# mariaalfaroc/omr_a2s_multimodal_transformer

Measured on AMD Instinct MI355X. Metric: training samples/sec, higher is better.
Workload: dtype bf16; 1 GPU; C2: image encoder (CNN) + 6-layer d_model=256 kern decoder, fwd+bwd+Adam, dropout on, teacher-forcing noise on; one sample = one score image + its token sequence; per_gpu_batch=32, global_batch=32, image=256x2048x1, seq_len=512, layers=6, d_model=256, vocab=6997, parallelism=dp1

## Files before the change

omr_a2s_multimodal_transformer_amd/csrc/gemm.hip:

```cpp
#include <type_traits>

#include "omr_common.h"
#include "omr_hip.h"

#include "gemm_steps.h"

namespace {

struct TileId { int m, n, split; bool valid; };
__device__ __forceinline__ TileId tile_of_block(const GemmArgs& g, int L) {
    const int slot = L >> 3;
    const long J = ((long)(slot / g.chunk) * 8 + (L & 7)) * g.chunk + slot % g.chunk;
    TileId t;
    t.valid = J < g.total;
    t.n = (int)(J % g.nt);
    t.m = (int)((J / g.nt) % g.mt);
    t.split = (int)(J / ((long)g.nt * g.mt));
    return t;
}

constexpr int BM = 128, BN = 128;

}

typedef unsigned char fp8;
typedef __attribute__((ext_vector_type(16))) unsigned char u8x16;
template <> struct Frag<fp8> {
    typedef u8x16 type;
    static constexpr int N = 16;
};
template <> __device__ __forceinline__ fp8 from_f32<fp8>(float x) { return (fp8)(__builtin_amdgcn_cvt_pk_fp8_f32(x, 0.f, 0, false) & 0xff); }
__device__ __forceinline__ float to_f32(fp8 x) { return __builtin_amdgcn_cvt_f32_fp8((int)x, 0); }
__device__ __forceinline__ void mma32(f32x16& acc, u8x16 a, u8x16 b) {
    long a2[2], b2[2];
    __builtin_memcpy(a2, &a, 16);
    __builtin_memcpy(b2, &b, 16);
    acc = __builtin_amdgcn_mfma_f32_32x32x16_fp8_fp8(a2[0], b2[0], acc, 0, 0, 0);
    acc = __builtin_amdgcn_mfma_f32_32x32x16_fp8_fp8(a2[1], b2[1], acc, 0, 0, 0);
}

namespace {

template <typename T> struct GemmCfg {
    static constexpr int VEC = Frag<T>::N;
    static constexpr int BK = 4 * KStep<T>::value;
    static constexpr int PITCH = BK + VEC;
    static constexpr int CHUNKS_PER_ROW = BK / VEC;
    static constexpr int NCH = BM * BK / VEC / 256;
    static constexpr int TPITCH = 128 + 32;
    static constexpr int OP_ELEMS = (BM * PITCH > BK * TPITCH) ? BM * PITCH : BK * TPITCH;
    static constexpr int CPITCH = 64 + 8;
    static constexpr int LDS_ELEMS = (2 * OP_ELEMS > 4 * 64 * CPITCH) ? 2 * OP_ELEMS : 4 * 64 * CPITCH;
};
template <typename T, bool TR> struct UseTrRead { static constexpr bool value = TR && std::is_same<T, bf16>::value; };

template <typename T> __device__ __forceinline__ typename Frag<T>::type load_chunk_guard(
    const T* p, int valid)
{
    typedef typename Frag<T>::type F;
    if (valid <= 0) return frag_zero<T>();
    F v = *reinterpret_cast<const F*>(p);
    if (valid < Frag<T>::N) {
#pragma unroll
        for (int i = 0; i < Frag<T>::N; ++i)
            if (i >= valid) v[i] = from_f32<T>(0.f);
    }
    return v;
}

template <typename T, bool TR> struct Stager {
    typedef GemmCfg<T> Cfg;
    typedef typename Frag<T>::type F;
    F r[Cfg::NCH];
    __device__ __forceinline__ void load(const T* src, long ld, int row0, int nrows, int k0, int kend, int tid) {
#pragma unroll
        for (int i = 0; i < Cfg::NCH; ++i) {
            const int c = tid + i * 256;
            if (!TR) {
                const int row = c / Cfg::CHUNKS_PER_ROW, kc = (c % Cfg::CHUNKS_PER_ROW) * Cfg::VEC;
                const int gr = row0 + row, gk = k0 + kc;
                r[i] = (gr < nrows) ? load_chunk_guard<T>(src + (long)gr * ld + gk, kend - gk) : frag_zero<T>();
            } else {
                constexpr int CPR = 128 / Cfg::VEC;
                const int k = c / CPR, rc = (c % CPR) * Cfg::VEC;
                const int gk = k0 + k, gr = row0 + rc;
                r[i] = (gk < kend) ? load_chunk_guard<T>(src + (long)gk * ld + gr, nrows - gr) : frag_zero<T>();
            }
        }
    }
    __device__ __forceinline__ void store(T* lds, int tid) {
#pragma unroll
        for (int i = 0; i < Cfg::NCH; ++i) {
            const int c = tid + i * 256;
            if (!TR) {
                const int row = c / Cfg::CHUNKS_PER_ROW, kc = (c % Cfg::CHUNKS_PER_ROW) * Cfg::VEC;
                *reinterpret_cast<F*>(lds + row * Cfg::PITCH + kc) = r[i];
            } else {
                constexpr int CPR = 128 / Cfg::VEC;
                const int k = c / CPR, rc = (c % CPR) * Cfg::VEC;
                if constexpr (UseTrRead<T, TR>::value) {
                    *reinterpret_cast<F*>(lds + k * Cfg::TPITCH + rc) = r[i];
                } else {
#pragma unroll
                    for (int e = 0; e < Cfg::VEC; ++e) lds[(rc + e) * Cfg::PITCH + k] = r[i][e];
                }
            }
        }
    }
    __device__ __forceinline__ void add_colsum(float (&cs)[Cfg::VEC]) {
#pragma unroll
        for (int i = 0; i < Cfg::NCH; ++i)
#pragma unroll
            for (int e = 0; e < Cfg::VEC; ++e) cs[e] += to_f32(r[i][e]);
    }
};

template <typename T, bool TR>
__device__ __forceinline__ typename Frag<T>::type load_frag(const T* lds, int row0, int ks, int lane) {
    typedef GemmCfg<T> Cfg;
    typedef typename Frag<T>::type F;
    if constexpr (UseTrRead<T, TR>::value) {
        const int q = (lane & 15) >> 2, col = row0 + ((lane >> 4) & 1) * 16 + (lane & 3) * 4, k = ks + 8 * (lane >> 5) + q;
        return tr_frag_bf16(lds + k * Cfg::TPITCH + col, 4 * Cfg::TPITCH * (int)sizeof(T));
    } else {
        return *reinterpret_cast<const F*>(&lds[(row0 + (lane & 31)) * Cfg::PITCH + ks + (lane >> 5) * Cfg::VEC]);
    }
}

template <typename T, typename TC, bool TA, bool TB, bool FULLK>
__device__ __forceinline__ void gemm_body(const GemmArgs& g, const int block_index) {
    typedef GemmCfg<T> Cfg;
    typedef typename Frag<T>::type F;
    constexpr bool SWAP = std::is_same<TC, bf16>::value && std::is_same<T, bf16>::value;
    __shared__ __attribute__((aligned(16))) T smem[Cfg::LDS_ELEMS];
    T* As = smem;
    T* Bs = smem + Cfg::OP_ELEMS;

    const int tid = threadIdx.x, lane = tid & 63, wave = tid >> 6;
    const int wm = wave >> 1, wn = wave & 1;
    const TileId tile = tile_of_block(g, block_index);
    if (!tile.valid) return;
    const int m0 = tile.m * BM, n0 = tile.n * BN;
    const int kbeg = tile.split * g.ksplit_len;
    const int kend = min(g.K, kbeg + g.ksplit_len);
    const T* A = (const T*)g.A;
    const T* B = (const T*)g.B + grp_delta(g, 1, n0) * g.ldb;

    __shared__ __attribute__((aligned(16))) float sbias[BN];
    if constexpr (SWAP) {
        if (tid < BN) {
            const float* bp = g.bias ? g.bias + grp_delta(g, 1, n0) : nullptr;
            sbias[tid] = (bp != nullptr && tile.split == 0 && n0 + tid < g.N) ? bp[n0 + tid] : 0.f;
        }
    }

    f32x16 acc[2][2];
    acc_clear(acc);
    float cs[Cfg::VEC];
#pragma unroll
    for (int e = 0; e < Cfg::VEC; ++e) cs[e] = 0.f;
    const bool do_cs = TA && g.colsum_a != nullptr && tile.n == 0;
    auto mma_slab = [&]() {
#pragma unroll
        for (int ks = 0; ks < Cfg::BK; ks += KStep<T>::value) {
            F a[2], b[2];
#pragma unroll
            for (int i = 0; i < 2; ++i) a[i] = load_frag<T, TA>(As, wm * 64 + i * 32, ks, lane);
#pragma unroll
            for (int j = 0; j < 2; ++j) b[j] = load_frag<T, TB>(Bs, wn * 64 + j * 32, ks, lane);
#pragma unroll
            for (int i = 0; i < 2; ++i)
#pragma unroll
                for (int j = 0; j < 2; ++j) {
                    if constexpr (SWAP) mma32(acc[i][j], b[j], a[i]);
                    else mma32(acc[i][j], a[i], b[j]);
                }
        }
    };
    if constexpr (FULLK) {
        Stager<T, TA> fa[4];
        Stager<T, TB> fb[4];
        const int nk = (kend - kbeg + Cfg::BK - 1) / Cfg::BK;
#pragma unroll
        for (int sl = 0; sl < 4; ++sl)
            if (sl < nk) {
                fa[sl].load(A, g.lda, m0, g.M, kbeg + sl * Cfg::BK, kend, tid);
                fb[sl].load(B + grp_delta(g, 2, kbeg + sl * Cfg::BK) * g.ldb, g.ldb, n0, g.N, kbeg + sl * Cfg::BK, kend, tid);
            }
#pragma unroll
        for (int sl = 0; sl < 4; ++sl)
            if (sl < nk) {
                if (sl) __syncthreads();
                fa[sl].store(As, tid);
                fb[sl].store(Bs, tid);
                __syncthreads();
                mma_slab();
            }
        __syncthreads();
    } else {
        Stager<T, TA> sa;
        Stager<T, TB> sb;
        sa.load(A, g.lda, m0, g.M, kbeg, kend, tid);
        sb.load(B + grp_delta(g, 2, kbeg) * g.ldb, g.ldb, n0, g.N, kbeg, kend, tid);
        if (do_cs) sa.add_colsum(cs);
        sa.store(As, tid);
        sb.store(Bs, tid);
        __syncthreads();

        for (int k0 = kbeg; k0 < kend; k0 += Cfg::BK) {
            const bool more = (k0 + Cfg::BK) < kend;
            if (more) {
                sa.load(A, g.lda, m0, g.M, k0 + Cfg::BK, kend, tid);
                sb.load(B + grp_delta(g, 2, k0 + Cfg::BK) * g.ldb, g.ldb, n0, g.N, k0 + Cfg::BK, kend, tid);
            }
            mma_slab();
            __syncthreads();
            if (more) {
                if (do_cs) sa.add_colsum(cs);
                sa.store(As, tid);
                sb.store(Bs, tid);
                __syncthreads();
            }
        }
    }

    if (do_cs) {
        constexpr int CPR = 128 / Cfg::VEC;
        float* red = reinterpret_cast<float*>(smem);
        if (tid < 128) red[tid] = 0.f;
        __syncthreads();
        const int ml = (tid % CPR) * Cfg::VEC;
#pragma unroll
        for (int e = 0; e < Cfg::VEC; ++e) atomicAdd(&red[ml + e], cs[e]);
        __syncthreads();
        if (tid < 128 && m0 + tid < g.M) atomicAdd(&g.colsum_a[m0 + tid + grp_delta(g, 3, m0)], red[tid]);
        __syncthreads();
    }

    TC* C = (TC*)g.C + grp_delta(g, 3, m0) * g.ldc;
    const float* biasp = g.bias ? g.bias + grp_delta(g, 1, n0) : nullptr;
    if constexpr (SWAP) {
        T* Cs = smem + wave * (64 * Cfg::CPITCH);
        const int hsel = 4 * (lane >> 5);
#pragma unroll
        for (int j = 0; j < 2; ++j) {
            float bv[16];
#pragma unroll
            for (int q = 0; q < 4; ++q) {
                const f32x4 b4 = *reinterpret_cast<const f32x4*>(&sbias[wn * 64 + j * 32 + 8 * q + hsel]);
                bv[4 * q] = b4[0]; bv[4 * q + 1] = b4[1]; bv[4 * q + 2] = b4[2]; bv[4 * q + 3] = b4[3];
            }
#pragma unroll
            for (int i = 0; i < 2; ++i) {
                T* crow = Cs + (i * 32 + (lane & 31)) * Cfg::CPITCH + j * 32 + hsel;
#pragma unroll
                for (int q = 0; q < 4; ++q)
                    *reinterpret_cast<bf16x4*>(crow + 8 * q) = pack_ct4(acc[i][j], q, [&](float v, int e) {
                        v = v + bv[4 * q + e];
                        if (g.relu) v = fmaxf(v, 0.f);
                        return v;
                    });
            }
        }
        const bool vec_ok = (g.ldc % 8) == 0 && (((uintptr_t)C) & 15) == 0;
#pragma unroll
        for (int it = 0; it < 8; ++it) {
            const int c = lane + it * 64, row = c >> 3, kc = (c & 7) * 8;
            const int gr = m0 + wm * 64 + row, gc = n0 + wn * 64 + kc;
            if (gr >= g.M || gc >= g.N) continue;
            bf16x8 v = *reinterpret_cast<const bf16x8*>(Cs + row * Cfg::CPITCH + kc);
            if (g.drop_thresh) {
#pragma unroll
                for (int e = 0; e < 8; ++e)
                    v[e] = drop_keep(g.drop_seed, (uint64_t)((long)gr * g.ldc + gc + e), g.drop_thresh) ? (bf16)((float)v[e] * g.drop_scale) : (bf16)0.f;
            }
            TC* dst = C + (long)gr * g.ldc + gc;
            if (vec_ok && gc + 8 <= g.N && !g.accum) {
                *reinterpret_cast<bf16x8*>(dst) = v;
            } else {
#pragma unroll
                for (int e = 0; e < 8; ++e)
                    if (gc + e < g.N) dst[e] = g.accum ? (bf16)((float)dst[e] + (float)v[e]) : v[e];
            }
        }
    } else {
        const int col_l = lane & 31;
#pragma unroll
        for (int j = 0; j < 2; ++j) {
            const int col = n0 + wn * 64 + j * 32 + col_l;
            if (col >= g.N) continue;
            const float bv = (biasp != nullptr && tile.split == 0) ? biasp[col] : 0.f;
#pragma unroll
            for (int i = 0; i < 2; ++i) {
#pragma unroll
                for (int r = 0; r < 16; ++r) {
                    const int row = m0 + wm * 64 + i * 32 + acc_row(r, lane);
                    if (row >= g.M) continue;
                    float v = acc[i][j][r];
                    if constexpr (std::is_same<T, fp8>::value) v *= g.scale_a[row] * g.scale_b[col];
                    v += bv;
                    if (g.relu) v = fmaxf(v, 0.f);
                    if constexpr (!TA) {
                        if (g.drop_thresh) v = drop_keep(g.drop_seed, (uint64_t)((long)row * g.ldc + col), g.drop_thresh) ? to_f32(from_f32<TC>(v)) * g.drop_scale : 0.f;
                    }
                    TC* dst = C + (long)row * g.ldc + col;
                    if (g.atomic) {
                        if constexpr (sizeof(TC) == 4) atomicAdd((float*)dst, v);
                    } else if (g.accum) {
                        *dst = from_f32<TC>(to_f32(*dst) + v);
                    } else {
                        *dst = from_f32<TC>(v);
                    }
                }
            }
        }
    }
}

template <typename T, typename TC, bool TA, bool TB, bool FULLK>
__global__ __launch_bounds__(256) void gemm_kernel(GemmArgs g) {
    gemm_body<T, TC, TA, TB, FULLK>(g, blockIdx.x);
}

struct GemmPlan { int ksplit_len, splits, mt, nt, total, chunk, blocks; };
template <typename D, typename S> __host__ __device__ __forceinline__ void put_plan(D& d, const S& s) {
    d.ksplit_len = s.ksplit_len; d.mt = s.mt; d.nt = s.nt; d.chunk = s.chunk; d.total = s.total;
}

struct DwProb {
    const void* A; const void* B; float* C; float* colsum;
    int M, N, K, ksplit_len; int lda, ldb, ldc, block0; int nt, mt, chunk, total; int grp, grp_stride, grp_base, pad;
};
constexpr int DW_MAX = 24;
struct DwGroup { int nprob, pad; DwProb p[DW_MAX]; };
static_assert(sizeof(DwGroup) == 2312, "the table travels as kernel arguments: DwProb stays the compact record, not a GemmArgs (160 bytes each)");

template <typename T>
__global__ __launch_bounds__(256) void gemm_dw_grouped_kernel(DwGroup grp) {
    int pi = 0;
    for (int i = 1; i < grp.nprob; ++i) pi = ((int)blockIdx.x >= grp.p[i].block0) ? i : pi;
    const DwProb& q = grp.p[pi];
    GemmArgs g;
    g.A = q.A; g.B = q.B; g.C = q.C; g.M = q.M; g.N = q.N; g.K = q.K; g.lda = q.lda; g.ldb = q.ldb; g.ldc = q.ldc;
    g.accum = 1; g.atomic = 1; g.colsum_a = q.colsum;
    put_plan(g, q);
    g.grp = q.grp; g.grp_stride = q.grp_stride; g.grp_base = q.grp_base; g.grp_operand = q.grp ? 3 : 0;
    gemm_body<T, float, true, true, false>(g, (int)blockIdx.x - q.block0);
}

GemmPlan gemm_plan(int M, int N, int K, int bk, int want_splits) {
    GemmPlan p;
    p.ksplit_len = cdiv(cdiv(K, want_splits), bk) * bk;
    p.splits = cdiv(K, p.ksplit_len);
    p.mt = cdiv(M, BM); p.nt = cdiv(N, BN);
    p.total = p.nt * p.mt * p.splits;
    p.chunk = p.splits > 1 ? p.nt * p.mt : p.nt;
    p.blocks = cdiv(p.total / p.chunk, 8) * 8 * p.chunk;
    return p;
}

template <typename T, typename TC> int launch(GemmArgs g, int ta, int tb, const GemmPlan& p, hipStream_t s) {
    put_plan(g, p);
    constexpr bool CAN_FULLK = !std::is_same<T, fp8>::value;
    const bool fullk = CAN_FULLK && !ta && p.splits == 1 && g.K <= 4 * GemmCfg<T>::BK;
    void (*kernel)(GemmArgs) = nullptr;
    if constexpr (!CAN_FULLK) kernel = (ta || tb) ? nullptr : gemm_kernel<T, TC, false, false, false>;
    else if (ta) kernel = tb ? gemm_kernel<T, TC, true, true, false> : gemm_kernel<T, TC, true, false, false>;
    else if (tb) kernel = fullk ? gemm_kernel<T, TC, false, true, true> : gemm_kernel<T, TC, false, true, false>;
    else kernel = fullk ? gemm_kernel<T, TC, false, false, true> : gemm_kernel<T, TC, false, false, false>;
    if (!kernel) return OMR_ERR_UNSUPPORTED;
    hipLaunchKernelGGL(kernel, dim3((unsigned)p.blocks), dim3(256), 0, s, g);
    OMR_CHECK_LAUNCH();
    return OMR_OK;
}

}

extern "C" int omr_gemm(int dtype, int c_dtype, int transA, int transB, int M, int N, int K, const void* A, long lda,
                        const void* B, long ldb, void* C, long ldc, const float* bias, int relu, int accumulate,
                        int split_k, float* colsum_a, float drop_p, unsigned long long drop_seed, int row_group, int row_group_stride,
                        int row_group_base, int row_group_operand, void* stream) {
    if (M <= 0 || N <= 0 || K <= 0 || !A || !B || !C) return OMR_ERR_ARG;
    const int vec = dtype == OMR_BF16 ? 8 : 4;
    if (lda % vec || ldb % vec) return OMR_ERR_ARG;
    if (((uintptr_t)A & 15) || ((uintptr_t)B & 15)) return OMR_ERR_ARG;
    if (split_k < 1) split_k = 1;
    if (split_k > 1 && c_dtype != OMR_F32) return OMR_ERR_ARG;
    GemmArgs g;
    g.A = A; g.B = B; g.C = C; g.bias = bias; g.M = M; g.N = N; g.K = K; g.lda = lda; g.ldb = ldb; g.ldc = ldc;
    g.relu = relu; g.accum = accumulate; g.atomic = split_k > 1; g.colsum_a = colsum_a;
    if (drop_p < 0.f || drop_p >= 1.f || (drop_p > 0.f && (split_k > 1 || accumulate || transA))) return OMR_ERR_ARG;
    if (row_group_operand) {
        if (row_group_operand < 1 || row_group_operand > 3 || row_group <= 0 || row_group % 128 || row_group_stride < row_group || row_group_base < 0) return OMR_ERR_ARG;
        if ((row_group_operand == 2 && !transB) || (row_group_operand == 1 && transB)) return OMR_ERR_ARG;
        g.grp = row_group; g.grp_stride = row_group_stride; g.grp_base = row_group_base; g.grp_operand = row_group_operand;
    }
    g.drop_thresh = OMR_DROP_THRESH16(drop_p); g.drop_scale = 1.f / (1.f - drop_p); g.drop_seed = drop_seed;
    if (colsum_a && !transA) return OMR_ERR_ARG;
    const GemmPlan plan = gemm_plan(M, N, K, dtype == OMR_BF16 ? 64 : 32, split_k);
    hipStream_t s = (hipStream_t)stream;
    const GemmCall call = {dtype, c_dtype, transA, transB, plan.splits, drop_p};
    int rc = omr_gemm_panel_bf16(call, g, s);
    if (rc == OMR_ERR_UNSUPPORTED) rc = omr_gemm_tall_bf16(call, g, s);
    if (rc != OMR_ERR_UNSUPPORTED) return rc;
    if (dtype == OMR_BF16) {
        if (c_dtype == OMR_BF16) return launch<bf16, bf16>(g, transA, transB, plan, s);
        return launch<bf16, float>(g, transA, transB, plan, s);
    } else if (dtype == OMR_F32) {
        if (c_dtype != OMR_F32) return OMR_ERR_UNSUPPORTED;
        return launch<float, float>(g, transA, transB, plan, s);
    }
    return OMR_ERR_UNSUPPORTED;
}

extern "C" int omr_linear_wgrad_grouped(int dtype, int nprob, const omr_dw_problem* probs, void* stream) {
    if (nprob <= 0 || !probs) return OMR_ERR_ARG;
    if (dtype != OMR_BF16 && dtype != OMR_F32) return OMR_ERR_UNSUPPORTED;
    const int vec = dtype == OMR_BF16 ? 8 : 4, bk = dtype == OMR_BF16 ? 64 : 32;
    long tiles_total = 0;
    for (int i = 0; i < nprob; ++i) tiles_total += (long)cdiv(probs[i].n_out, BM) * cdiv(probs[i].n_in, BN);
    hipStream_t s = (hipStream_t)stream;
    for (int base = 0; base < nprob; base += DW_MAX) {
        DwGroup grp;
        grp.nprob = nprob - base < DW_MAX ? nprob - base : DW_MAX; grp.pad = 0;
        int block0 = 0;
        for (int i = 0; i < grp.nprob; ++i) {
            const omr_dw_problem& q = probs[base + i];
            if (!q.dy || !q.x || !q.dw || q.rows <= 0 || q.n_out <= 0 || q.n_in <= 0) return OMR_ERR_ARG;
            if (q.ld_dy % vec || q.ld_x % vec || ((uintptr_t)q.dy & 15) || ((uintptr_t)q.x & 15)) return OMR_ERR_ARG;
            if (q.row_group && (q.row_group % 128 || q.row_group_stride < q.row_group || q.row_group_base < 0)) return OMR_ERR_ARG;
            DwProb& d = grp.p[i];
            d.A = q.dy; d.B = q.x; d.C = q.dw; d.colsum = q.db;
            d.M = q.n_out; d.N = q.n_in; d.K = q.rows; d.lda = (int)q.ld_dy; d.ldb = (int)q.ld_x; d.ldc = (int)q.ld_dw;
            long want = (2048L + tiles_total - 1) / tiles_total;
            long maxs = (q.rows + 511) / 512;
            if (want > maxs) want = maxs;
            if (want < 1) want = 1;
            const GemmPlan plan = gemm_plan(d.M, d.N, d.K, bk, (int)want);
            put_plan(d, plan);
            d.block0 = block0;
            block0 += plan.blocks;
            d.grp = q.row_group; d.grp_stride = q.row_group_stride; d.grp_base = q.row_group_base; d.pad = 0;
        }
        if (dtype == OMR_BF16) hipLaunchKernelGGL((gemm_dw_grouped_kernel<bf16>), dim3((unsigned)block0), dim3(256), 0, s, grp);
        else hipLaunchKernelGGL((gemm_dw_grouped_kernel<float>), dim3((unsigned)block0), dim3(256), 0, s, grp);
        OMR_CHECK_LAUNCH();
    }
    return OMR_OK;
}

namespace {
template <typename T>
__global__ __launch_bounds__(256) void quantize_rows_fp8_kernel(const T* __restrict__ x, long ldx, fp8* __restrict__ q, long ldq, float* __restrict__ scale,
                                                                int M, int K) {
    const int lane = threadIdx.x & 63;
    const long row = blockIdx.x * (long)(blockDim.x >> 6) + (threadIdx.x >> 6);
    if (row >= M) return;
    const T* xr = x + row * ldx;
    float mx = 0.f;
    for (int k = lane; k < K; k += 64) mx = fmaxf(mx, fabsf(to_f32(xr[k])));
    mx = wave_max(mx);
    const float sc = mx > 0.f ? mx / 448.f : 1.f;
    for (int k = lane; k < K; k += 64) q[row * ldq + k] = from_f32<fp8>(to_f32(xr[k]) / sc);
    if (lane == 0) scale[row] = sc;
}
}

extern "C" int omr_quantize_rows_fp8(int dtype, const void* x, long ldx, unsigned char* q, long ldq, float* scale, int M, int K, void* stream) {
    if (M <= 0 || K <= 0 || !x || !q || !scale || ldx < K || ldq < K) return OMR_ERR_ARG;
    hipStream_t s = (hipStream_t)stream;
    if (dtype == OMR_BF16) hipLaunchKernelGGL((quantize_rows_fp8_kernel<bf16>), cdiv(M, 4), 256, 0, s, (const bf16*)x, ldx, q, ldq, scale, M, K);
    else if (dtype == OMR_F32) hipLaunchKernelGGL((quantize_rows_fp8_kernel<float>), cdiv(M, 4), 256, 0, s, (const float*)x, ldx, q, ldq, scale, M, K);
    else return OMR_ERR_UNSUPPORTED;
    OMR_CHECK_LAUNCH();
    return OMR_OK;
}

extern "C" int omr_gemm_fp8(int c_dtype, int M, int N, int K, const unsigned char* A8, long lda, const float* scale_a, const unsigned char* W8, long ldb,
                            const float* scale_w, void* C, long ldc, const float* bias, int relu, void* stream) {
    if (M <= 0 || N <= 0 || K <= 0 || !A8 || !W8 || !C || !scale_a || !scale_w) return OMR_ERR_ARG;
    if (lda % 16 || ldb % 16 || ((uintptr_t)A8 & 15) || ((uintptr_t)W8 & 15)) return OMR_ERR_ARG;
    GemmArgs g;
    g.A = A8; g.B = W8; g.C = C; g.bias = bias; g.M = M; g.N = N; g.K = K; g.lda = lda; g.ldb = ldb; g.ldc = ldc;
    g.relu = relu; g.scale_a = scale_a; g.scale_b = scale_w;
    const GemmPlan plan = gemm_plan(M, N, K, GemmCfg<fp8>::BK, 1);
    hipStream_t s = (hipStream_t)stream;
    if (c_dtype == OMR_BF16) return launch<fp8, bf16>(g, 0, 0, plan, s);
    if (c_dtype == OMR_F32) return launch<fp8, float>(g, 0, 0, plan, s);
    return OMR_ERR_UNSUPPORTED;
}
```

omr_a2s_multimodal_transformer_amd/csrc/gemm_args.h:

```cpp
#pragma once
#include <hip/hip_runtime.h>

struct GemmArgs {
    const void* A = nullptr; const void* B = nullptr; void* C = nullptr; const float* bias = nullptr;
    int M = 0, N = 0, K = 0; long lda = 0, ldb = 0, ldc = 0;
    int relu = 0, accum = 0, atomic = 0, ksplit_len = 0;
    float* colsum_a = nullptr;
    int mt = 0, nt = 0, chunk = 0, total = 0;
    unsigned drop_thresh = 0; float drop_scale = 1.f; unsigned long long drop_seed = 0;
    int grp = 0, grp_stride = 0, grp_base = 0, grp_operand = 0;
    const float* scale_a = nullptr; const float* scale_b = nullptr;
};
static_assert(sizeof(GemmArgs) == 160, "GemmArgs travels as kernel arguments");

struct GemmCall { int dtype, c_dtype, trans_a, trans_b, splits; float drop_p; };
int omr_gemm_panel_bf16(const GemmCall& call, const GemmArgs& g, hipStream_t s);
int omr_gemm_tall_bf16(const GemmCall& call, const GemmArgs& g, hipStream_t s);
```

Before: 1391 samples/s.

## Add stream-K grouped weight-gradient kernel for n_in=256 bf16 problems

Routes bf16 weight-gradient problems with n_in equal to 256 to a new persistent kernel. It splits the flattened (problem, output tile, k-tile) item space evenly across at most one workgroup per CU. Each 1024-thread workgroup double-buffers 64-row slabs of dy and x in 128 KB of LDS via async DMA, accumulates a 256x256 tile with MFMA, and flushes partial results and the bias column-sum with atomics at tile boundaries. The aim is better load balance and fewer small launches than the 128x128 split-K grouped kernel for the decoder's d_model=256 linears. In exchange it relies on fp32 atomics, which make the summation order nondeterministic, and on high LDS use per workgroup.

```diff
diff --git a/omr_a2s_multimodal_transformer_amd/csrc/gemm.hip b/omr_a2s_multimodal_transformer_amd/csrc/gemm.hip
--- a/omr_a2s_multimodal_transformer_amd/csrc/gemm.hip
+++ b/omr_a2s_multimodal_transformer_amd/csrc/gemm.hip
@@ -1,4 +1,5 @@
 #include <type_traits>
+#include <vector>
 
 #include "omr_common.h"
 #include "omr_hip.h"
@@ -417,18 +418,25 @@
     if (nprob <= 0 || !probs) return OMR_ERR_ARG;
     if (dtype != OMR_BF16 && dtype != OMR_F32) return OMR_ERR_UNSUPPORTED;
     const int vec = dtype == OMR_BF16 ? 8 : 4, bk = dtype == OMR_BF16 ? 64 : 32;
+    for (int i = 0; i < nprob; ++i) {
+        const omr_dw_problem& q = probs[i];
+        if (!q.dy || !q.x || !q.dw || q.rows <= 0 || q.n_out <= 0 || q.n_in <= 0) return OMR_ERR_ARG;
+        if (q.ld_dy % vec || q.ld_x % vec || ((uintptr_t)q.dy & 15) || ((uintptr_t)q.x & 15)) return OMR_ERR_ARG;
+        if (q.row_group && (q.row_group % 128 || q.row_group_stride < q.row_group || q.row_group_base < 0)) return OMR_ERR_ARG;
+    }
+    hipStream_t s = (hipStream_t)stream;
+    std::vector<omr_dw_problem> rest((size_t)nprob);
+    const int rc = omr_dw_stream_bf16(dtype, nprob, probs, rest.data(), &nprob, s);
+    if (rc != OMR_OK) return rc;
+    probs = rest.data();
     long tiles_total = 0;
     for (int i = 0; i < nprob; ++i) tiles_total += (long)cdiv(probs[i].n_out, BM) * cdiv(probs[i].n_in, BN);
-    hipStream_t s = (hipStream_t)stream;
     for (int base = 0; base < nprob; base += DW_MAX) {
         DwGroup grp;
         grp.nprob = nprob - base < DW_MAX ? nprob - base : DW_MAX; grp.pad = 0;
         int block0 = 0;
         for (int i = 0; i < grp.nprob; ++i) {
             const omr_dw_problem& q = probs[base + i];
-            if (!q.dy || !q.x || !q.dw || q.rows <= 0 || q.n_out <= 0 || q.n_in <= 0) return OMR_ERR_ARG;
-            if (q.ld_dy % vec || q.ld_x % vec || ((uintptr_t)q.dy & 15) || ((uintptr_t)q.x & 15)) return OMR_ERR_ARG;
-            if (q.row_group && (q.row_group % 128 || q.row_group_stride < q.row_group || q.row_group_base < 0)) return OMR_ERR_ARG;
             DwProb& d = grp.p[i];
             d.A = q.dy; d.B = q.x; d.C = q.dw; d.colsum = q.db;
             d.M = q.n_out; d.N = q.n_in; d.K = q.rows; d.lda = (int)q.ld_dy; d.ldb = (int)q.ld_x; d.ldc = (int)q.ld_dw;
diff --git a/omr_a2s_multimodal_transformer_amd/csrc/gemm_args.h b/omr_a2s_multimodal_transformer_amd/csrc/gemm_args.h
--- a/omr_a2s_multimodal_transformer_amd/csrc/gemm_args.h
+++ b/omr_a2s_multimodal_transformer_amd/csrc/gemm_args.h
@@ -16,3 +16,6 @@
 struct GemmCall { int dtype, c_dtype, trans_a, trans_b, splits; float drop_p; };
 int omr_gemm_panel_bf16(const GemmCall& call, const GemmArgs& g, hipStream_t s);
 int omr_gemm_tall_bf16(const GemmCall& call, const GemmArgs& g, hipStream_t s);
+
+struct omr_dw_problem;
+int omr_dw_stream_bf16(int dtype, int nprob, const omr_dw_problem* probs, omr_dw_problem* rest, int* nrest, hipStream_t s);
diff --git a/omr_a2s_multimodal_transformer_amd/csrc/gemm_dw_stream.hip b/omr_a2s_multimodal_transformer_amd/csrc/gemm_dw_stream.hip
--- /dev/null
+++ b/omr_a2s_multimodal_transformer_amd/csrc/gemm_dw_stream.hip
@@ -0,0 +1,198 @@
+#include <climits>
+#include "omr_common.h"
+#include "omr_hip.h"
+#include "gemm_steps.h"
+#include "dma_common.h"
+#include "launch_setup.h"
+
+namespace {
+
+constexpr int TM = 256, NIN = 256;
+constexpr int BK = 64, KS = BK / 16;
+constexpr int ROWB = NIN * 2;
+constexpr int SLAB = BK * ROWB, STAGE = 2 * SLAB, SMEM = 2 * STAGE;
+constexpr int COPIES = BK / 2 / 16;
+constexpr int ITEMS_PER_WG = 8;
+static_assert(SMEM == 131072 && COPIES == 2, "two 64 KB stages, 2 + 2 copies per wave and k-tile");
+
+struct DwsProb {
+    const bf16* dy; const bf16* x; float* dw; float* db;
+    int rows, n_out, ld_dy, ld_x, ld_dw, grp, grp_stride, grp_base, item0, pad;
+};
+constexpr int DWS_MAX = 40;
+struct DwsTable { int nprob, nitems; DwsProb p[DWS_MAX]; };
+static_assert(sizeof(DwsProb) == 72 && sizeof(DwsTable) == 2888, "the table travels as kernel arguments (4 KB at the most)");
+
+struct Cursor { int p, t, kt, nk, tiles; };
+__device__ __forceinline__ void cursor_problem(Cursor& c, const DwsTable& tab, int p) {
+    c.p = p; c.nk = (tab.p[p].rows + BK - 1) / BK; c.tiles = (tab.p[p].n_out + TM - 1) / TM;
+}
+__device__ __forceinline__ void cursor_next(Cursor& c, const DwsTable& tab) {
+    if (++c.kt < c.nk) return;
+    c.kt = 0;
+    if (++c.t < c.tiles) return;
+    c.t = 0;
+    cursor_problem(c, tab, c.p + 1);
+}
+
+__device__ __forceinline__ float sum8(bf16x8 f) {
+    const uint4 u = __builtin_bit_cast(uint4, f);
+    const unsigned w[4] = {u.x, u.y, u.z, u.w};
+    float s = 0.f;
+#pragma unroll
+    for (int e = 0; e < 4; ++e) s += __uint_as_float(w[e] << 16) + __uint_as_float(w[e] & 0xffff0000u);
+    return s;
+}
+
+__global__ __launch_bounds__(1024) void gemm_dw_grouped_stream_kernel(DwsTable tab) {
+    extern __shared__ __attribute__((aligned(16))) unsigned char smem[];
+    const int tid = threadIdx.x, lane = tid & 63, hh = lane >> 5, wave = __builtin_amdgcn_readfirstlane(tid >> 6), wm = wave >> 2, wn = wave & 3;
+    const unsigned lds0 = lds_address(smem);
+    const int G = (int)gridDim.x;
+    const int it0 = (int)((long)blockIdx.x * tab.nitems / G), it1 = (int)((long)(blockIdx.x + 1) * tab.nitems / G);
+    if (it0 >= it1) return;
+
+    const int q = (lane & 15) >> 2, pc = ((lane >> 4) & 1) * 16 + (lane & 3) * 4;
+    int d_off[2], x_off[2];
+#pragma unroll
+    for (int i = 0; i < 2; ++i) {
+        const int cd = wm * 64 + i * 32 + pc, cx = wn * 64 + i * 32 + pc;
+        d_off[i] = (8 * hh + q) * ROWB + (((cd >> 3) ^ (q << 2)) << 4) + (cd & 7) * 2;
+        x_off[i] = SLAB + (8 * hh + q) * ROWB + (((cx >> 3) ^ (q << 2)) << 4) + (cx & 7) * 2;
+    }
+    int kr[COPIES], cb[COPIES];
+#pragma unroll
+    for (int u = 0; u < COPIES; ++u) {
+        kr[u] = (COPIES * wave + u) * 2 + (lane >> 5);
+        cb[u] = (lane & 31) ^ ((kr[u] & 3) << 2);
+    }
+    auto issue = [&](const Cursor& c, int stage) {
+        const DwsProb& pr = tab.p[c.p];
+        const unsigned st = lds0 + stage * STAGE;
+        const int k0 = c.kt * BK, last_row = pr.rows - 1, last_chunk = ((pr.n_out + 7) >> 3) - 1, c0 = c.t * (TM / 8);
+#pragma unroll
+        for (int u = 0; u < COPIES; ++u) {
+            const long row = min(k0 + kr[u], last_row);
+            dma16(pr.dy + row * pr.ld_dy + min(c0 + cb[u], last_chunk) * 8, st + (COPIES * wave + u) * 1024);
+            dma16(pr.x + row * pr.ld_x + cb[u] * 8, st + SLAB + (COPIES * wave + u) * 1024);
+        }
+    };
+
+    Cursor cc;
+    {
+        int p = 0;
+        for (int i = 1; i < tab.nprob; ++i) p = (it0 >= tab.p[i].item0) ? i : p;
+        cursor_problem(cc, tab, p);
+        const int local = it0 - tab.p[p].item0;
+        cc.t = local / cc.nk; cc.kt = local % cc.nk;
+    }
+    Cursor ci = cc;
+
+    f32x16 acc[2][2];
+    acc_clear(acc);
+    const bool db_wave = wn == wm;
+    float dbs[2] = {0.f, 0.f};
+
+    issue(ci, 0);
+    for (int it = it0; it < it1; ++it) {
+        const int stage = (it - it0) & 1;
+        dma_wait_barrier<0>();
+        if (it + 1 < it1) { cursor_next(ci, tab); issue(ci, stage ^ 1); }
+        unsigned char* st = smem + stage * STAGE;
+        const int valid = tab.p[cc.p].rows - cc.kt * BK;
+        if (valid < BK) {
+#pragma unroll
+            for (int e = 0; e < 2 * SLAB / 16 / 1024; ++e) {
+                const int ch = tid + e * 1024;
+                if (((ch >> 5) & (BK - 1)) >= valid) *reinterpret_cast<uint4*>(st + ch * 16) = make_uint4(0, 0, 0, 0);
+            }
+            lds_barrier();
+        }
+#pragma unroll
+        for (int ks = 0; ks < KS; ++ks) {
+            bf16x8 df[2], xf[2];
+#pragma unroll
+            for (int i = 0; i < 2; ++i) df[i] = tr_frag_bf16(st + d_off[i] + ks * 16 * ROWB, 4 * ROWB);
+#pragma unroll
+            for (int j = 0; j < 2; ++j) xf[j] = tr_frag_bf16(st + x_off[j] + ks * 16 * ROWB, 4 * ROWB);
+#pragma unroll
+            for (int i = 0; i < 2; ++i)
+#pragma unroll
+                for (int j = 0; j < 2; ++j) mma32(acc[i][j], df[i], xf[j]);
+            if (db_wave) {
+#pragma unroll
+                for (int i = 0; i < 2; ++i) dbs[i] += sum8(df[i]);
+            }
+        }
+        const bool last = it + 1 == it1;
+        if (cc.kt + 1 == cc.nk || last) {
+            const DwsProb& pr = tab.p[cc.p];
+            const int m0 = cc.t * TM;
+            const long delta = pr.grp ? (long)(m0 / pr.grp) * (pr.grp_stride - pr.grp) + pr.grp_base : 0;
+            float* dwt = pr.dw + (m0 + delta) * (long)pr.ld_dw + wn * 64 + (lane & 31);
+            const int n_left = pr.n_out - m0;
+#pragma unroll
+            for (int i = 0; i < 2; ++i)
+#pragma unroll
+                for (int r = 0; r < 16; ++r) {
+                    const int ml = wm * 64 + i * 32 + (r >> 2) * 8 + hh * 4 + (r & 3);
+                    if (ml < n_left) {
+#pragma unroll
+                        for (int j = 0; j < 2; ++j) atomicAdd(dwt + (long)ml * pr.ld_dw + j * 32, acc[i][j][r]);
+                    }
+                }
+            acc_clear(acc);
+            if (db_wave) {
+#pragma unroll
+                for (int i = 0; i < 2; ++i) {
+                    const float v = dbs[i] + __shfl_xor(dbs[i], 32);
+                    const int ml = wm * 64 + i * 32 + (lane & 31);
+                    if (pr.db && hh == 0 && ml < n_left) atomicAdd(pr.db + m0 + delta + ml, v);
+                    dbs[i] = 0.f;
+                }
+            }
+        }
+        if (!last) cursor_next(cc, tab);
+    }
+}
+
+bool accepts(int dtype, const omr_dw_problem& q) {
+    if (dtype != OMR_BF16 || q.n_in != NIN || q.rows <= 0 || q.n_out <= 0) return false;
+    if (q.ld_dy % 8 || q.ld_x % 8 || ((uintptr_t)q.dy & 15) || ((uintptr_t)q.x & 15)) return false;
+    if (q.ld_dy < q.n_out || q.ld_x < NIN || q.ld_dw < NIN || q.ld_dy > INT_MAX || q.ld_x > INT_MAX || q.ld_dw > INT_MAX) return false;
+    if (q.row_group && q.row_group % TM) return false;
+    return (long)cdiv(q.n_out, TM) * cdiv(q.rows, BK) < (1L << 24);
+}
+
+}
+
+int omr_dw_stream_bf16(int dtype, int nprob, const omr_dw_problem* probs, omr_dw_problem* rest, int* nrest, hipStream_t s) {
+    *nrest = 0;
+    DwsTable tab;
+    tab.nprob = 0; tab.nitems = 0;
+    auto launch = [&]() -> int {
+        if (!tab.nprob) return OMR_OK;
+        static std::atomic<int> ready{0};
+        if (!omr_launch_setup(ready, (const void*)gemm_dw_grouped_stream_kernel, SMEM, true)) return OMR_ERR_LAUNCH;
+        const int want = tab.nitems / ITEMS_PER_WG, grid = want < 1 ? 1 : want > OMR_NUM_CU ? OMR_NUM_CU : want;
+        hipLaunchKernelGGL(gemm_dw_grouped_stream_kernel, dim3(grid), dim3(1024), SMEM, s, tab);
+        OMR_CHECK_LAUNCH();
+        tab.nprob = 0; tab.nitems = 0;
+        return OMR_OK;
+    };
+    for (int i = 0; i < nprob; ++i) {
+        const omr_dw_problem& q = probs[i];
+        if (!accepts(dtype, q)) { rest[(*nrest)++] = q; continue; }
+        const int items = cdiv(q.n_out, TM) * cdiv(q.rows, BK);
+        if (tab.nprob == DWS_MAX || tab.nitems + (long)items > INT_MAX / 2) {
+            const int rc = launch();
+            if (rc != OMR_OK) return rc;
+        }
+        DwsProb& d = tab.p[tab.nprob++];
+        d.dy = (const bf16*)q.dy; d.x = (const bf16*)q.x; d.dw = q.dw; d.db = q.db;
+        d.rows = q.rows; d.n_out = q.n_out; d.ld_dy = (int)q.ld_dy; d.ld_x = (int)q.ld_x; d.ld_dw = (int)q.ld_dw;
+        d.grp = q.row_group; d.grp_stride = q.row_group_stride; d.grp_base = q.row_group_base; d.item0 = tab.nitems; d.pad = 0;
+        tab.nitems += items;
+    }
+    return launch();
+}
```

Measured after the change: 1398 samples/s (median of 6 runs). No clear change (+0.5%).
